# pgriewank/SAMSIM

Hardware: AMD Instinct MI355X
Metric: column-timesteps/sec (higher is better)
Workload: dtype f64

## Files before the change

samsim_amd/csrc/samsim_probe.h:

```cpp
#ifndef SAMSIM_PROBE_H
#define SAMSIM_PROBE_H

#ifndef SAMSIM_STAMPS
#define SAMSIM_STAMPS 0
#endif
#ifdef SAMSIM_ISA_MARKS
#define ISA_MARK(name) asm volatile("; ISA_MARK " name)
#else
#define ISA_MARK(name) ((void)0)
#endif
#if SAMSIM_STAMPS
__device__ unsigned long long g_stamps[48];
extern "C" int samsim_debug_stamps(unsigned long long *out, int reset) {
  if (out && hipMemcpyFromSymbol(out, HIP_SYMBOL(g_stamps), sizeof(unsigned long long) * 48) != hipSuccess) return -1;
  if (reset) { unsigned long long z[48] = {0}; if (hipMemcpyToSymbol(HIP_SYMBOL(g_stamps), z, sizeof(z)) != hipSuccess) return -1; }
  return 0;
}
#endif

namespace {

#if SAMSIM_STAMPS
enum { ST_PRO = 0, ST_DFUSED, ST_DUNFUSED, ST_SURF, ST_UP, ST_POST, ST_HEAD, ST_TAIL,
       CT_WAVESTEPS = 8, CT_FUSED, CT_UNFUSED, CT_UP_TRIPS, CT_NEWTON_WAVE, CT_NEWTON_LANE, CT_LANES, CT_DOWN_TRIPS, CT_DRAIN_WAVE,
       CT_DRAIN_LANE, CT_DIRTY, CT_L_COUPLING, ST_U_HEAD = 20, ST_U_GETT, ST_U_TAIL, ST_D_A, ST_D_B,
       CT_L_FLOODP = 25, CT_L_IRREG, CT_L_DIRTY, CT_L_UNFUSED, CT_L_FLUSH3, CT_L_REGRID, CT_L_FREEBOARD,
       CT_REFILL = 32, CT_ROWS, CT_ROWS_STILL, CT_ODD_LANES, CT_ODD_WAVES, CT_ODD_EVALS_WAVE, CT_LITE, ST_NSLOT = 48 };
struct Stamps {
  unsigned long long *acc;
  unsigned long long t0;
};
__device__ __forceinline__ bool st_leader() { return (int)__lane_id() == __ffsll((long long)__ballot(1)) - 1; }
__device__ __forceinline__ void st_mark(Stamps &st, int region) {
#if SAMSIM_STAMPS == 1
  const unsigned long long t = __builtin_amdgcn_s_memtime();
  if (st_leader()) st.acc[region] += t - st.t0;
  st.t0 = t;
#endif
}
__device__ __forceinline__ void st_count(Stamps &st, int counter, unsigned long long n = 1) {
#if SAMSIM_STAMPS == 2
  if (st_leader()) st.acc[counter] += n;
#endif
}
#define ST_MARK(r) st_mark(x.st, r)
#define ST_COUNT(cn, n) st_count(x.st, cn, n)
#else
#define ST_MARK(r) ((void)0)
#define ST_COUNT(cn, n) ((void)0)
#endif

}

#endif
```

samsim_amd/csrc/samsim_sweeps_fused.h:

```cpp
#ifndef SAMSIM_SWEEPS_FUSED_H
#define SAMSIM_SWEEPS_FUSED_H

namespace {


struct RayScan {
  double minp, stp, st;
  double bot, botterm, perm_bot, S_br_bot;
  double buoy_s, min_psi_s;
};
__device__ __forceinline__ void ray_scan_init(RayScan &r) {
  r.minp = 1.0e300; r.stp = 0.0; r.st = 0.0; r.bot = 0.0; r.botterm = 0.0; r.perm_bot = 0.0; r.S_br_bot = 0.0;
  r.buoy_s = 0.0; r.min_psi_s = 1.0e300;
}

struct Expelled { double psi_s, psi_l, psi_g, V_ex; };
__device__ __forceinline__ Expelled expulsion(double phi, double thick, double m, double rth) {
  Expelled e;
  const double V_s = m * phi * (1.0 / rho_s), V_l = m * (1.0 - phi) * (1.0 / rho_l);
  e.V_ex = dmax(V_l + V_s - thick, 0.0);
  e.psi_s = V_s * rth;
  e.psi_l = (V_l - e.V_ex) * rth;
  e.psi_g = (thick - V_l - V_s + e.V_ex) * rth;
  e.psi_l = dmax(e.psi_l, 0.0);
  e.psi_g = dmax(e.psi_g, 0.0);
  return e;
}

template <class K>
__device__ __forceinline__ void s1_layer(Col &c, const Ctx &x, int k, int Na, bool do_ray, double T, double phi, double S_bu,
                                         double m, double thick, double rth, RayScan &r, bool sparse_rows = false, const double *S_br_T = nullptr) {
  const samsim_config &g = x.p->cfg;
  const double S_br = S_br_T ? *S_br_T : S_br_clamped(x.salt, T, S_bu);
  const Expelled e = expulsion(phi, thick, m, rth);
  r.min_psi_s = dmin(r.min_psi_s, e.psi_s);
  r.buoy_s += e.psi_s * thick;
  if (k == 1) c.psi_l_top = e.psi_l;
  if (do_ray) {
    const double perm = x.p17 * pow_3p1(1000.0 * fabs(e.psi_l));
    if (k == Na) {
      r.S_br_bot = S_br;
      r.bot = thick * e.psi_s / psi_s_min;
      r.perm_bot = perm;
      r.botterm = r.bot / perm;
    } else {
      const double height = r.st + r.bot;
      r.minp = dmin(r.minp, perm);
      r.stp = r.stp + quot(thick, perm);
      r.st = r.st + thick;
      double ray;
      const double d_S_br = S_br - r.S_br_bot;
      if (CFG(harmonic_flag) == 2) {
        const double hp = (r.minp < x.p14) ? 0.0 : quot(r.st + r.bot, r.stp + r.botterm);
        ray = grav_f * rho_l * bbeta * d_S_br * height * hp;
      } else {
        ray = grav_f * rho_l * bbeta * d_S_br * height * dmin(r.minp, r.perm_bot);
      }
      ray = ray * (1.0 / (kappa_l * mu));
      ray = dmax(ray, 0.0);
      if (!sparse_rows) {
        LAYU(SAMSIM_A_RAY, k) = ray;
      } else if (k == 1 || x.ray_rows_all || wave_any(ray > ray_crit)) {
        LAYU(SAMSIM_A_RAY, k) = ray;
        x.rflag[(k - 1) >> 6] = x.rflag[(k - 1) >> 6] | (1ull << ((k - 1) & 63));
      }
    }
  }
}

template <class K>
__device__ __forceinline__ void flood_handover(Col &c, const Ctx &x, const RayScan &all, const RayScan &below_top, double thick_bottom) {
  const samsim_config &g = x.p->cfg;
  if (!(CFG(flood_flag) > 1 && c.Na > 1 && CL(m_snow) > all.buoy_s * (rho_l - rho_s))) return;
  SPEC(SP_FL_HP) = quot(all.st + all.bot, all.stp + all.botterm);
  SPEC(SP_FL_SALL) = all.st + thick_bottom;
  SPEC(SP_MINP) = below_top.minp; SPEC(SP_STP) = below_top.stp; SPEC(SP_ST) = below_top.st;
  SPEC(SP_BOT) = below_top.bot; SPEC(SP_BOTTERM) = below_top.botterm; SPEC(SP_SBR_BOT) = below_top.S_br_bot;
}

template <class K>
__device__ __forceinline__ void prologue_top_layer(Col &c, const Ctx &x) {
  const samsim_config &g = x.p->cfg;
  const int Na = c.Na;
  const bool do_ray = (CFG(grav_flag) >= 2 && Na > 1);
  RayScan r;
  r.minp = SPEC(SP_MINP); r.stp = SPEC(SP_STP); r.st = SPEC(SP_ST);
  r.bot = SPEC(SP_BOT); r.botterm = SPEC(SP_BOTTERM); r.perm_bot = SPEC(SP_PERM_BOT);
  r.S_br_bot = SPEC(SP_SBR_BOT); r.buoy_s = SPEC(SP_BUOY_S); r.min_psi_s = SPEC(SP_MIN_PSI_S);
  const RayScan r_below_top = r;
  const double H_abs = LAY(SAMSIM_A_H_ABS, 1), m = LAY(SAMSIM_A_M, 1), thick = LAY(SAMSIM_A_THICK, 1);
  double S_abs = LAY(SAMSIM_A_S_ABS, 1);
  if (S_abs < 0.0) { S_abs = 0.0; LAY(SAMSIM_A_S_ABS, 1) = S_abs; }
  double S_bu, H;
  per_mass(S_abs, H_abs, m, S_bu, H);
  if (K::general && CFG(prescribe_flag) == 2) LAY(SAMSIM_A_S_BU, 1) = S_abs / m;
  const double T_test = (Na > 1) ? LAY(SAMSIM_A_T, 2) : g.T_bottom;
  double T, phi = 0.0;
  const int rc = getT_chain(x.salt, H, S_bu, T_test, T, phi);
  LAY(SAMSIM_A_T, 1) = T;
  LAY(SAMSIM_A_PHI, 1) = phi;
  s1_layer<K>(c, x, 1, Na, do_ray, T, phi, S_bu, m, thick, recip(thick), r);
  if (do_ray && CFG(flood_flag) > 1 && CL(m_snow) > r.buoy_s * (rho_l - rho_s)) {
    THICK_RULE_INIT(tr);
    flood_handover<K>(c, x, r, r_below_top, THICK_AT(tr, Na));
  }
  c.neg_psi = r.min_psi_s < 0.0;
  c.buoy_s = r.buoy_s;
  if (rc) STOPC(rc, 1);
}

template <class K>
__device__ RARE void sweep_beer(Col &c, const Ctx &x, double beer0) {
  const samsim_config &g = x.p->cfg;
  const int Na = c.Na;
  if (!wave_any(beer0 != 0.0)) { c.frad = 0.0; return; }
  if ((c.flags & COLF_REGULAR) != 0) {
    const int n0 = __builtin_amdgcn_readfirstlane(Na);
    const bool same = !wave_any(Na != n0);
    const int kend = same ? n0 : wave_max(Na);
    const int b0 = g.n_top, b1 = g.n_top + g.n_middle;
    double temp2 = beer0, frad = 0.0;
#pragma unroll 1
    for (int st = 0; st < 4; ++st) {
      const int klo = st == 0 ? 1 : (st == 1 ? 2 : (st == 2 ? b0 + 1 : b1 + 1));
      const int khi_s = st == 0 ? 1 : (st == 1 ? b0 : (st == 2 ? b1 : kend));
      if (klo > kend) break;
      if (klo > khi_s) continue;
      const int khi = khi_s < kend ? khi_s : kend;
      const double thick = st == 0 ? LAYU(SAMSIM_A_THICK, 1) : (st == 2 ? LAYU(SAMSIM_A_THICK, g.n_top + 1) : g.thick_0);
      const double e = exp(-extinc * thick);
      if (same) {
        const int kmul = khi < kend ? khi : kend - 1;
        for (int k = klo; k <= kmul; ++k) temp2 = temp2 * e;
        if (khi == kend) frad = temp2 - temp2 * e;
      } else {
        for (int k = klo; k <= khi; ++k) {
          const double t = temp2 * e;
          if (k == Na) frad = temp2 - t;
          temp2 = t;
        }
      }
    }
    c.frad = frad;
  } else {
    double temp2 = beer0, e = 0.0, th_prev = -1.0;
    for (int k = 1; k <= Na; ++k) {
      const double thick = LAYU(SAMSIM_A_THICK, k);
      if (thick != th_prev) { e = exp(-extinc * thick); th_prev = thick; }
      if (k == Na) c.frad = temp2 - temp2 * e;
      temp2 = temp2 * e;
    }
  }
}

__device__ __forceinline__ double heat_conductance(double psi_s, double psi_l, double rth) {
  return (2.0 * (psi_s * k_s + psi_l * k_l)) * rth;
}
__device__ __forceinline__ double heat_flux_between(double dT, double g_a, double g_b) {
  return quot(dT * (g_a * g_b), g_a + g_b);
}

__device__ __forceinline__ double out_of_row(double v) {
#if defined(__HIP_DEVICE_COMPILE__)
  double r;
  asm volatile("v_mov_b64 %0, %1" : "=v"(r) : "v"(v));
  return r;
#else
  return v;
#endif
}

template <class K>
__device__ __forceinline__ void sweep_down_fused(Col &c, const Ctx &x, bool store_default, bool decide_psi, bool &surface_done,
                                                 bool couple, bool late_rad, double time, int tc, bool do_beer) {
  const samsim_config &g = x.p->cfg;
  const Salt &s = x.salt;
  const int Na = c.Na;
  const double dt = g.dt;
  double heat_loss = 0.0, cum = 0.0, sum_before = 0.0, sum_after = 0.0, minS = 1.0e300;
  double fb_a2 = 0.0, fb_g2 = 0.0;
  int stop_layer = 0;
  bool store_psi = true;
  double g_up = 0.0, flq_up = 0.0;
  double esum = 0.0;

  struct Ld { double T, S_abs, m, H_abs, ray; };
  struct Raw { double T, S_abs, m, S_bu, S_br, H_abs, ray, H; };
  auto load_ld = [&](int j) -> Ld {
    Ld r;
    r.T = LAYU_LD(SAMSIM_A_T, j);
    r.S_abs = LAYU_LD(SAMSIM_A_S_ABS, j);
    r.m = LAYU_LD(SAMSIM_A_M, j);
    r.H_abs = LAYU_LD(SAMSIM_A_H_ABS, j);
    r.ray = (j <= Na - 1 && ray_row_valid(c, x, j)) ? LAYU(SAMSIM_A_RAY, j) : 0.0;
    return r;
  };
  auto finish = [&](const Ld &l, int j) -> Raw {
    Raw r;
    r.T = l.T; r.S_abs = l.S_abs; r.m = l.m; r.H_abs = l.H_abs; r.ray = l.ray;
    per_mass(r.S_abs, r.H_abs, r.m, r.S_bu, r.H);
    r.S_br = S_br_clamped(s, r.T, r.S_bu);
    return r;
  };
  auto S_br_below = [&](const Ld &l) -> double {
    double S_bu, H;
    per_mass(l.S_abs, l.H_abs, l.m, S_bu, H);
    return S_br_clamped(s, l.T, S_bu);
  };
  struct Lay { double T, SA, mA, S_abs, H_abs, m, flup; bool ch; };

  double flm_j = 0.0;
  double T_up = 0.0, S_br_up = 0.0, S_abs_up = 0.0;
  const int N = c.N;
  Raw raw = finish(load_ld(1), 1);
  Ld ahead = load_ld(2), ahead2 = ahead;
  Lay prev = {0, 0, 1, 0, 0, 0, 0, true};
  double flup_pp = 0.0;
  auto layer = [&](const int j, const Ld &below, const double thick, const double rth, auto last_tag, auto first_tag) {
    constexpr bool LAST = decltype(last_tag)::value, FIRST = decltype(first_tag)::value;
    if (!LAST && !FIRST) { ISA_MARK("D_LAYER_A"); }
    double H_abs = raw.H_abs;
    const Expelled ex = expulsion(phi_from_T(s, raw.H, raw.S_bu, raw.S_br), thick, raw.m, rth);
    const double V_ex = ex.V_ex;
    double psi_g = ex.psi_g, m = raw.m, S_abs = raw.S_abs;
    const double T = raw.T, S_br = raw.S_br;
    double flm_next;
    if (j == 1 || psi_g < (double)0.001f) {
      flm_next = (j == 1) ? -V_ex * rho_l : -V_ex * rho_l + flm_j;
    } else {
      flm_next = -dmax((V_ex - psi_g * thick) * rho_l, 0.0);
      psi_g = dmax(quot(psi_g * thick - V_ex, thick), 0.0);
    }
    if (!FIRST) { fb_a2 += ex.psi_s * thick; fb_g2 += psi_g * thick; }
    if (store_psi || j == 1) {
      LAYU(SAMSIM_A_PSI_S, j) = ex.psi_s;
      LAYU(SAMSIM_A_PSI_L, j) = ex.psi_l;
      LAYU(SAMSIM_A_PSI_G, j) = psi_g;
    }
    const bool flooded_here = FIRST && (c.flags & COLF_FLOODED) != 0;
    const double th_l = flooded_here ? LAYU(SAMSIM_A_THICK, 1) : thick;
    const double gj = heat_conductance(ex.psi_s, ex.psi_l, flooded_here ? recip(th_l) : rth);
    const double flq = (j >= 2) ? heat_flux_between(T - prev.T, g_up, gj) : 0.0;
    if (j == 2) c.flq2 = flq;
    m = m + flm_next - flm_j;
    if (flm_next < 0.0) {
      H_abs = H_abs + flm_next * T * c_l;
      S_abs = S_abs + dmax(flm_next * S_br, -S_abs);
    }
    if (flm_j < 0.0) {
      H_abs = H_abs - flm_j * T_up * c_l;
      S_abs = S_abs - dmax(flm_j * S_br_up, -S_abs_up);
    }
    bool ch = LAST || (flm_next < 0.0) || (flm_j < 0.0);
#if SAMSIM_STAMPS == 2
    if (!LAST && !FIRST) {
      ST_COUNT(CT_ROWS, 1);
      if (__ballot(flm_next < 0.0 || flm_j < 0.0) == 0ull) ST_COUNT(CT_ROWS_STILL, 1);
    }
#endif
    const double SA = S_abs, mA = m;
    S_br_up = S_br;
    flm_j = flm_next;
    double Tl = T;
    if (FIRST && couple) {
      double phi1 = LAYU(SAMSIM_A_PHI, 1);
      const double S_bu1 = S_abs / m;
      LAYU(SAMSIM_A_S_BU, 1) = S_bu1;
      const int rcc = snow_coupling_core<K>(c, x, H_abs, m, S_bu1, Tl, phi1);
      LAYU(SAMSIM_A_T, 1) = Tl;
      LAYU(SAMSIM_A_PHI, 1) = phi1;
      if (rcc && !c.status) { c.status = rcc; x.err_step[c.col] = c.step + 1; x.err_layer[c.col] = 1; }
    }
    if (flooded_here) {
      S_abs = SPEC(SP_FLD_S1); H_abs = SPEC(SP_FLD_H1); m = SPEC(SP_FLD_M1);
      ch = true;
      c.flags &= ~COLF_FLOODED;
    }
    if (LAST) {
      if (psi_g > 0.0) {
        const double t2 = psi_g * thick * rho_l;
        m = m + t2;
        S_abs = S_abs + t2 * x.S_bu_bottom;
        H_abs = H_abs + t2 * c_l * g.T_bottom;
      }
      if (c.flags & COLF_FLOOD_DEEP) {
        S_abs = S_abs + SPEC(SP_FL_HP);
        H_abs = H_abs + SPEC(SP_FL_SALL);
        c.flags &= ~COLF_FLOOD_DEEP;
      }
      if (CFG(turb_flag) == 2) {
        const double turb = Turb_A * exp(Turb_B * (-ocean_density<K>(x) + func_density(T, quot(S_abs, m)))) * dt;
        S_abs = S_abs - turb * (S_abs / m - x.S_bu_bottom);
      }
    }
    if (!LAST && !FIRST) { ISA_MARK("D_LAYER_B"); }
    ST_MARK(ST_D_A);
    sum_before += S_abs;
    double flup = cum;
    if (!LAST) {
      const double ray = raw.ray;
      if (ray > ray_crit && S_br > S_br_below(below)) {
        const double psi_s = ex.psi_s;
        if (psi_s > 0.001 && (flooded_here ? quot(S_abs, m) : quot(SA, mA)) > 0.1) {
          ST_COUNT(CT_DRAIN_WAVE, 1);
          ST_COUNT(CT_DRAIN_LANE, (unsigned long long)__popcll(__ballot(1)));
          const double psi_l = ex.psi_l;
          double flux = x_grav * (ray - ray_crit) * dt * th_l;
          flux = dmin(flux, psi_l * rho_l * th_l);
          S_abs = S_abs - flux * S_br;
          if (S_abs < 0.0 && !stop_layer) stop_layer = j;
          CL(grav_temp) = CL(grav_temp) + flux * Tl;
          H_abs = H_abs - flux * c_l * Tl;
          heat_loss = heat_loss + flux * c_l * Tl;
          cum = cum + flux;
          flup = dmin(cum, psi_l * rho_l * th_l);
          ch = true;
        }
      }
    }
    sum_after += S_abs;
#if defined(__HIP_DEVICE_COMPILE__)
    asm volatile("" : "+v"(sum_before), "+v"(sum_after));
#endif
    if (!LAST && !FIRST) { ISA_MARK("D_LAYER_C"); }
    if (j > 1) {
      if (prev.flup > 0.0) {
        prev.H_abs = prev.H_abs + prev.flup * T * c_l;
        prev.S_abs = prev.S_abs + dmin(prev.flup * S_br_clamped(s, T, quot(SA, mA)), S_abs);
        prev.ch = true;
      }
      if (flup_pp > 0.0) {
        prev.H_abs = prev.H_abs - flup_pp * prev.T * c_l;
        prev.S_abs = prev.S_abs - dmin(flup_pp * S_br_clamped(s, prev.T, quot(prev.SA, prev.mA)), prev.S_abs);
        prev.ch = true;
      }
      if (j - 1 >= 2) {
        const double H_b = prev.H_abs;
        prev.H_abs = prev.H_abs + (flq - flq_up) * dt;
        prev.H_abs = prev.H_abs + c.frad * dt;
        esum += H_b - prev.H_abs;
      }
      if (wave_any(prev.ch)) {
        LAYU(SAMSIM_A_M, j - 1) = prev.m;
        LAYU(SAMSIM_A_S_ABS, j - 1) = prev.S_abs;
      }
      LAYU(SAMSIM_A_H_ABS, j - 1) = prev.H_abs;
      minS = dmin(minS, prev.S_abs);
      flup_pp = prev.flup;
    }
    g_up = gj; flq_up = flq;
    T_up = out_of_row(T); S_abs_up = out_of_row(SA);
    prev.T = FIRST ? out_of_row(Tl) : T_up; prev.SA = S_abs_up; prev.mA = mA; prev.S_abs = out_of_row(S_abs); prev.H_abs = out_of_row(H_abs);
    prev.m = m; prev.flup = flup; prev.ch = ch;
    if (!LAST && !FIRST) { ISA_MARK("D_LAYER_END"); }
    ST_MARK(ST_D_B);
  };
  const int jmax = wave_max(Na);
  auto request = [&](const int j) { ahead2 = load_ld(j + 2 <= N ? j + 2 : N); };
  auto advance = [&](const int j) { raw = finish(ahead, j + 1); ahead = ahead2; };
  const double thick1 = (c.flags & COLF_FLOODED) ? SPEC(SP_FLD_TH1_BEFORE) : LAYU(SAMSIM_A_THICK, 1);
  if (1 < Na) { request(1); layer(1, ahead, thick1, recip(thick1), std::false_type{}, std::true_type{}); advance(1); }
  if (2 < Na) { request(2); layer(2, ahead, g.thick_0, recip(g.thick_0), std::false_type{}, std::false_type{}); advance(2); }
  if (late_rad) {
    const double beer0 = radiation_header<K>(c, x, time, tc);
    c.frad = 0.0;
    if (do_beer) sweep_beer<K>(c, x, beer0);
  }
  if (decide_psi && Na >= 3) {
    surface_flux<K>(c, x);
    surface_done = true;
    const double thick_min = g.thick_min;
    const double Tf = func_T_freeze(quot(LAYU(SAMSIM_A_S_ABS, 1), LAYU(SAMSIM_A_M, 1)), CFG(salt_flag), x.tf_c3);
    bool snow_wet = false;
    if (CL(thick_snow) > 0.0) {
      const double H_new = CL(H_abs_snow) + (CL(fl_Q1) - CL(fl_Q_snow)) * dt;
      snow_wet = !(CL(thick_snow) >= thick_min) || !(H_new / CL(m_snow) <= -latent_heat);
    }
    store_psi = store_default || LAYU(SAMSIM_A_PSI_S, 1) < psi_s_top_min || CL(T_top) >= Tf || snow_wet || CL(melt_thick_snow) > 0.0;
  } else {
    store_psi = store_default || decide_psi;
  }
  c.psi_full = store_psi;
  {
    const int b0 = g.n_top, b1 = g.n_top + g.n_middle;
    Ld ahead3 = ahead;
    auto single = [&](const int j, const double th_s, const double rth_s) {
      ahead2 = load_ld(j + 2 <= N ? j + 2 : N);
      layer(j, ahead, th_s, rth_s, std::false_type{}, std::false_type{});
      raw = finish(ahead, j + 1);
      ahead = ahead2;
    };
    int j = 3;
    for (int stretch = 0; stretch < 3; ++stretch) {
      const int hi_s = stretch == 0 ? b0 : (stretch == 1 ? b1 : N);
      const int hi = hi_s < jmax - 1 ? hi_s : jmax - 1;
      const double th_s = stretch == 1 ? LAYU(SAMSIM_A_THICK, g.n_top + 1) : g.thick_0, rth_s = recip(th_s);
      for (; j + 2 <= hi; j += 3) {
        ISA_MARK("D_ITER_BEGIN");
        ST_MARK(ST_DFUSED);
        if (j + 2 < Na) {
          ST_COUNT(CT_DOWN_TRIPS, 3);
          ahead2 = load_ld(j + 2 <= N ? j + 2 : N);
          layer(j, ahead, th_s, rth_s, std::false_type{}, std::false_type{});
          raw = finish(ahead, j + 1);
          ahead3 = load_ld(j + 3 <= N ? j + 3 : N);
          layer(j + 1, ahead2, th_s, rth_s, std::false_type{}, std::false_type{});
          raw = finish(ahead2, j + 2);
          ahead = load_ld(j + 4 <= N ? j + 4 : N);
          layer(j + 2, ahead3, th_s, rth_s, std::false_type{}, std::false_type{});
          raw = finish(ahead3, j + 3);
        } else if (j < Na) {
          ISA_MARK("D_RARE_BEGIN");
          ST_COUNT(CT_DOWN_TRIPS, 1);
          single(j, th_s, rth_s);
          if (j + 1 < Na) { ST_COUNT(CT_DOWN_TRIPS, 1); single(j + 1, th_s, rth_s); }
        }
        ISA_MARK("D_ITER_END");
      }
      for (; j <= hi; ++j) {
        if (j < Na) single(j, th_s, rth_s);
      }
    }
  }
  const double thick_Na = (Na > g.n_top && Na <= g.n_top + g.n_middle) ? LAYU(SAMSIM_A_THICK, g.n_top + 1) : g.thick_0;
  layer(Na, ahead, thick_Na, recip(thick_Na), std::true_type{}, std::false_type{});
  if (prev.flup > 0.0) {
    prev.H_abs = prev.H_abs + prev.flup * g.T_bottom * c_l;
    prev.S_abs = prev.S_abs + dmin(prev.flup * S_br_clamped(s, g.T_bottom, x.S_bu_bottom), x.S_bu_bottom * 2000.0);
  }
  if (flup_pp > 0.0) {
    prev.H_abs = prev.H_abs - flup_pp * prev.T * c_l;
    prev.S_abs = prev.S_abs - dmin(flup_pp * S_br_clamped(s, prev.T, quot(prev.SA, prev.mA)), prev.S_abs);
  }
  CL(grav_drain) = CL(grav_drain) + prev.flup;
  if (CFG(grav_heat_flag) == 2) prev.H_abs = prev.H_abs + heat_loss - prev.flup * c_l * g.T_bottom;
  {
    const double H_b = prev.H_abs;
    prev.H_abs = prev.H_abs + (c.fl_q_bottom - flq_up) * dt;
    prev.H_abs = prev.H_abs + c.frad * dt;
    c.esum = esum + (H_b - prev.H_abs);
  }
  LAYU(SAMSIM_A_M, Na) = prev.m;
  LAYU(SAMSIM_A_S_ABS, Na) = prev.S_abs;
  LAYU(SAMSIM_A_H_ABS, Na) = prev.H_abs;
  minS = dmin(minS, prev.S_abs);
  if (store_psi) { SPEC(SP_FB_A2) = fb_a2; SPEC(SP_FB_G2) = fb_g2; }
  CL(grav_salt) = CL(grav_salt) + sum_before;
  CL(grav_salt) = CL(grav_salt) - sum_after;
  if (stop_layer) STOPC(21234, stop_layer);
  if (minS < 0.0) STOPC(1337, 0);
}

template <class K>
__device__ __forceinline__ void sweep_up_fused(Col &c, const Ctx &x, long long col, bool next_is_output, bool store_phi) {
  const samsim_config &g = x.p->cfg;
  const Salt &s = x.salt;
  const int Na = c.Na;
  const double dt = g.dt, thick_min = g.thick_min;
  const bool thin_snow = (CL(thick_snow) >= thick_min / 100.0 && CL(thick_snow) < thick_min);
  const bool do_ray = (CFG(grav_flag) >= 2 && Na > 1);
  const bool keep_ray = next_is_output && col >= x.out_col0 && col < x.out_col0 + x.out_ncols;
  const double H_abs_snow_before = CL(H_abs_snow);
  double esum = c.esum;
  double T_test = g.T_bottom;
  int rc = 0, rc_layer = 0;
  RayScan r;
  ray_scan_init(r);
  if (keep_ray) {
    const size_t oc = (size_t)(col - x.out_col0), on = (size_t)x.out_ncols;
    for (int k = 1; k <= c.N - 1; ++k) x.out_lay[((size_t)SAMSIM_A_RAY * c.N + (k - 1)) * on + oc] = LAYU(SAMSIM_A_RAY, k);
  }
  for (int w = 0; w <= (c.N - 1) >> 6; ++w) x.rflag[w] = 0ull;
  __builtin_amdgcn_wave_barrier();
  if (do_ray && Na <= c.N - 1 && x.ray_rows_all) LAYU(SAMSIM_A_RAY, Na) = 0.0;
  struct UL { double th, H, m, S; };
  const bool regular_wave = !wave_any((c.flags & COLF_REGULAR) == 0);
  UL cur, nxt, nn;
  bool alive = true, neg_salt = false;
  auto body = [&](const int k, const UL &row, const double th_k, const double rth_k, auto top_tag, auto lite_tag) {
    constexpr bool TOP = decltype(top_tag)::value;
    constexpr bool LITE = decltype(lite_tag)::value;
    const double H_k = row.H, m_k = row.m, S_k = row.S;
    double H_abs = H_k;
    const double m = m_k;
    if (TOP) {
      const double flq_below = (Na >= 2) ? c.flq2 : c.fl_q_bottom;
      const double H_b = H_abs;
      H_abs = H_abs + (flq_below - CL(fl_Q1)) * dt;
      H_abs = H_abs + c.frad * dt;
      if (thin_snow) {
        CL(H_abs_snow) = CL(H_abs_snow) - CL(fl_Q_snow) * dt;
        LAYU(SAMSIM_A_H_ABS, 1) = H_abs;
        snow_coupling<K>(c, x);
        if (c.status) { alive = false; return; }
        H_abs = LAYU(SAMSIM_A_H_ABS, 1);
      } else if (CL(thick_snow) >= thick_min) {
        CL(H_abs_snow) = CL(H_abs_snow) + (CL(fl_Q1) - CL(fl_Q_snow)) * dt;
      }
      esum += H_b - H_abs;
      LAYU(SAMSIM_A_H_ABS, 1) = H_abs;
    }
    double S_abs = S_k;
    double S_bu, H;
    per_mass(S_abs, H_abs, m, S_bu, H);
    double T, phi = 0.0, S_br_T = 0.0;
    if (!TOP) { ISA_MARK("U_GETT_BEGIN"); }
    ST_MARK(ST_U_HEAD);
#if SAMSIM_STAMPS == 2
    int evals = 1;
    int rr = TOP ? getT(s, H, S_bu, T_test, T, phi, &evals) : getT_chain<LITE>(s, H, S_bu, T_test, T, phi, &evals, LITE ? nullptr : &S_br_T);
    {
      const bool was_odd = (evals >> 30) & 1;
      const int redo = (evals >> 16) & 0x3fff;
      evals &= 0xffff;
      const unsigned long long om = __ballot(was_odd);
      if (om) { ST_COUNT(CT_ODD_LANES, (unsigned long long)__popcll(om)); ST_COUNT(CT_ODD_WAVES, 1); ST_COUNT(CT_ODD_EVALS_WAVE, (unsigned long long)wave_max(redo)); }
    }
    ST_COUNT(CT_UP_TRIPS, 1);
    ST_COUNT(CT_NEWTON_WAVE, (unsigned long long)wave_max(evals));
    { int tot = 0; unsigned long long mk = __ballot(1); while (mk) { const int ln = __ffsll((long long)mk) - 1; tot += __builtin_amdgcn_readlane(evals, ln); mk &= mk - 1; }
      ST_COUNT(CT_NEWTON_LANE, (unsigned long long)tot); }
#else
    int rr = TOP ? getT(s, H, S_bu, T_test, T, phi) : getT_chain<LITE>(s, H, S_bu, T_test, T, phi, nullptr, LITE ? nullptr : &S_br_T);
#endif
    if (!TOP) { ISA_MARK("U_GETT_END"); }
    ST_MARK(ST_U_GETT);
    if (rr && !rc) { rc = rr; rc_layer = k; }
    T_test = T;
    LAYU(SAMSIM_A_T, k) = T;
    if (store_phi || TOP || k >= Na - 1) LAYU(SAMSIM_A_PHI, k) = phi;
    if (!TOP && !LITE) {
      neg_salt = neg_salt || (S_abs < 0.0);
      s1_layer<K>(c, x, k, Na, do_ray, T, phi, S_bu, m, th_k, rth_k, r, true, &S_br_T);
    }
    ST_MARK(ST_U_TAIL);
  };
  const int kmax = wave_max(Na);
  auto load3 = [&](int j) -> UL { UL u; u.th = 0.0; u.H = LAYU_LD(SAMSIM_A_H_ABS, j); u.m = LAYU_LD(SAMSIM_A_M, j); u.S = LAYU_LD(SAMSIM_A_S_ABS, j); return u; };
  auto load4 = [&](int j) -> UL { UL u = load3(j); u.th = LAYU(SAMSIM_A_THICK, j); return u; };
  auto layers = [&](auto lite_tag) {
  if (regular_wave) {
    const int kc = kmax >= 2 ? kmax - 1 : 1;
    UL a = load3(kmax), b = load3(kc), d = b;
    auto one = [&](const int k, const UL &row, UL &req, const double th_s, const double rth_s) {
      req = load3(k >= 3 ? k - 2 : 1);
      if (k <= Na) body(k, row, th_s, rth_s, std::false_type{}, lite_tag);
    };
    const int b0 = g.n_top, b1 = g.n_top + g.n_middle;
    int k = kmax;
    for (int stretch = 0; stretch < 3; ++stretch) {
      const int klo = stretch == 0 ? b1 + 1 : (stretch == 1 ? b0 + 1 : 2);
      const double th_s = stretch == 1 ? LAYU(SAMSIM_A_THICK, g.n_top + 1) : g.thick_0, rth_s = recip(th_s);
      for (; k - 2 >= klo; k -= 3) {
        ISA_MARK("U_ITER_BEGIN");
        ST_MARK(ST_UP);
        one(k, a, d, th_s, rth_s);
        ISA_MARK("U_LAYER_2");
        one(k - 1, b, a, th_s, rth_s);
        ISA_MARK("U_LAYER_3");
        one(k - 2, d, b, th_s, rth_s);
        ISA_MARK("U_ITER_END");
      }
      for (; k >= klo; --k) {
        ISA_MARK("U_REST_BEGIN");
        ST_MARK(ST_UP);
        one(k, a, d, th_s, rth_s);
        a = b; b = d;
        ISA_MARK("U_REST_END");
      }
    }
    cur = a;
  } else {
    cur = load4(Na); nxt = load4(Na >= 2 ? Na - 1 : 1); nn = nxt;
    for (int k = kmax; k >= 2; --k) {
      if (k > Na) continue;
      nn = load4(k >= 3 ? k - 2 : 1);
      body(k, cur, cur.th, recip(cur.th), std::false_type{}, lite_tag);
      cur = nxt; nxt = nn;
    }
  }
  };
  const bool lite = K::fixed && CFG(flush_flag) == 5 && wave_any((c.flags & COLF_FLUSHED) != 0);
  if (lite) { ST_COUNT(CT_LITE, 1); layers(std::true_type{}); } else layers(std::false_type{});
  __builtin_amdgcn_wave_barrier();
  if (neg_salt || lite) c.flags |= COLF_DIRTY;
  body(1, cur, LAYU(SAMSIM_A_THICK, 1), 0.0, std::true_type{}, std::false_type{});
  if (!alive) return;
  if (!lite) {
  SPEC(SP_MINP) = r.minp; SPEC(SP_STP) = r.stp; SPEC(SP_ST) = r.st;
  SPEC(SP_BOT) = r.bot; SPEC(SP_BOTTERM) = r.botterm; SPEC(SP_PERM_BOT) = r.perm_bot;
  SPEC(SP_SBR_BOT) = r.S_br_bot; SPEC(SP_BUOY_S) = r.buoy_s; SPEC(SP_MIN_PSI_S) = r.min_psi_s;
  }
  double bal = esum + (H_abs_snow_before - CL(H_abs_snow));
  bal = bal + (double)Na * (c.frad * dt);
  if (thin_snow || CL(thick_snow) >= thick_min) bal = bal + c.fl_q_bottom * dt - CL(fl_Q_snow) * dt;
  else bal = bal + c.fl_q_bottom * dt - CL(fl_Q1) * dt;
  if (fabs(bal / dt) > 0.00001) STOPC(431, 0);
  if (rc) STOPC(rc, rc_layer);
}

}

#endif
```

samsim_amd/csrc/samsim_thermo.h:

```cpp
#ifndef SAMSIM_THERMO_H
#define SAMSIM_THERMO_H

namespace {

#include "samsim_div.h"
#if defined(__HIP_DEVICE_COMPILE__)
__device__ __forceinline__ double dmax(double a, double b) {
  double r;
  if (__builtin_constant_p(b) && b == 0.0) asm("v_max_f64 %0, %1, 0" : "=v"(r) : "v"(a));
  else asm("v_max_f64 %0, %1, %2" : "=v"(r) : "v"(a), "v"(b));
  return r;
}
__device__ __forceinline__ double dmin(double a, double b) {
  double r;
  asm("v_min_f64 %0, %1, %2" : "=v"(r) : "v"(a), "v"(b));
  return r;
}
#else
__device__ __forceinline__ double dmax(double a, double b) { return a > b ? a : b; }
__device__ __forceinline__ double dmin(double a, double b) { return a < b ? a : b; }
#endif
#if defined(__HIP_DEVICE_COMPILE__)
__device__ __forceinline__ double fma_c(double a, double b, double c_const) {
  double r;
  asm("v_fma_f64 %0, %1, %2, %3" : "=v"(r) : "v"(a), "v"(b), "s"(c_const));
  return r;
}
__device__ __forceinline__ double max_c(double a, double c_const) {
  double r;
  asm("v_max_f64 %0, %1, %2" : "=v"(r) : "v"(a), "s"(c_const));
  return r;
}
#else
__device__ __forceinline__ double fma_c(double a, double b, double c_const) { return __builtin_fma(a, b, c_const); }
__device__ __forceinline__ double max_c(double a, double c_const) { return a > c_const ? a : c_const; }
#endif
__device__ __forceinline__ void per_mass(double S_abs, double H_abs, double m, double &S_bu, double &H) {
  const double rm = recip(m);
  S_bu = S_abs * rm;
  H = H_abs * rm;
}

__device__ __forceinline__ double S_br_poly(const Salt &s, double T) {
  return T * (s.c2 + T * (s.c3 + T * s.c4));
}
__device__ __forceinline__ double S_br_clamped(const Salt &s, double T, double S_bu) {
  double v = S_br_poly(s, T);
  return dmax(v, S_bu);
}
__device__ __forceinline__ double ddT_S_br(const Salt &s, double T) {
  const double T_crit = -20.0;
  double d = s.d2 + 2.0 * s.d3 * T + 3.0 * s.d4 * (T * T);
  if (T < T_crit) d = s.d2 + 2.0 * s.d3 * T_crit + 3.0 * s.d4 * (T_crit * T_crit);
  return d;
}

__device__ __forceinline__ void newton_terms(const Salt &s, double H, double S_bu, double T_0, double sb, double sb_floor,
                                             double &f, double &ddT_f) {
  if (sb > 0.0001) {
    const double inv = recip(sb);
    f = -latent_heat - H + latent_heat * S_bu * inv + c_s * T_0 + c_s_beta * T_0 * T_0 / 2.0;
    ddT_f = c_s + c_s_beta * T_0 - latent_heat * S_bu * ddT_S_br(s, T_0) * (inv * inv);
    return;
  }
  f = -latent_heat - H + latent_heat * S_bu / dmax(sb, sb_floor) + c_s * T_0 + c_s_beta * T_0 * T_0 / 2.0;
  ddT_f = c_s + c_s_beta * T_0 - latent_heat * S_bu * ddT_S_br(s, T_0) / dmax(sb * sb, 0.0000000001);
}

struct NewtonConsts { double c3, cs, d3x2; };
__device__ __forceinline__ NewtonConsts newton_consts(const Salt &s) {
  NewtonConsts n = {s.c3, c_s, 2.0 * s.d3};
#if defined(__HIP_DEVICE_COMPILE__)
  asm volatile("" : "+v"(n.c3), "+v"(n.cs), "+v"(n.d3x2));
#endif
  return n;
}
__device__ __forceinline__ void newton_eval(const Salt &s, const NewtonConsts &n, double A0, double LS, double T_0, double &T_new, bool &more, bool &ok) {
  const double sbf = T_0 * fma_c(T_0, __builtin_fma(T_0, s.c4, n.c3), s.c2);
  const double sb2 = sbf * sbf;
  const double A = __builtin_fma(T_0, __builtin_fma(T_0, 0.5 * c_s_beta, n.cs), A0);
  const double B = __builtin_fma(c_s_beta, T_0, n.cs);
  const double num = __builtin_fma(A, sb2, LS * sbf);
  const double Tc = max_c(T_0, -20.0);
  const double dd = fma_c(Tc, __builtin_fma(Tc, 3.0 * s.d4, n.d3x2), s.d2);
  const double den = __builtin_fma(B, sb2, -(LS * dd));
  T_new = T_0 - quot(num, den);
  more = fabs(num) > sb2;
  ok = sbf > 0.0001;
}

__device__ __forceinline__ bool newton_step(const Salt &s, double H, double S_bu, double T_0, double sb_floor, double &T_new) {
  {
    bool more, ok;
    double Tn;
    newton_eval(s, newton_consts(s), -latent_heat - H, latent_heat * S_bu, T_0, Tn, more, ok);
    if (ok) { T_new = Tn; return more; }
  }
  const double sb = S_br_poly(s, T_0);
  double f, ddT_f;
  newton_terms(s, H, S_bu, T_0, sb, sb_floor, f, ddT_f);
  T_new = T_0 - quot(f, ddT_f);
  return fabs(f) > 1.0;
}

__device__ __forceinline__ double T_liquid(double H) {
  return H * (1.0 / c_l);
}

__device__ __forceinline__ double T_freeze_of(const Salt &s, double S_bu) {
  double T_fr = -1.0;
  while (fabs(S_br_poly(s, T_fr) / S_bu - 1.0) > (double)0.0001f) {
    const double t0 = T_fr;
    T_fr = t0 - (S_br_poly(s, t0) - S_bu) / ddT_S_br(s, t0);
  }
  return T_fr;
}

__device__ __forceinline__ int getT(const Salt &s, double H, double S_bu, double T_in, double &T_out, double &phi_out, int *evals = nullptr) {
  double T = T_liquid(H), phi = phi_out;
  int rc = 0;
  if (S_br_clamped(s, T, S_bu) > S_bu && S_bu > 0.001) {
    double T_fr = 0.0, T_0;
    bool have_T_fr = false;
    T_0 = T_in;
    bool more = newton_step(s, H, S_bu, T_0, 0.000000001, T);
    int i = 0;
    while (more) {
      T_0 = T;
      if (T_0 > 0.0 || T_0 < -200.0) {
        if (!have_T_fr) {
          T_fr = T_freeze_of(s, S_bu);
          have_T_fr = true;
        }
        T_0 = T_fr;
      }
      more = newton_step(s, H, S_bu, T_0, 0.0000000001, T);
#if SAMSIM_STAMPS == 2
      if (evals) *evals += 1;
#endif
      if (++i == 260) { rc = 99; break; }
    }
    phi = 1.0 - quot(S_bu, S_br_clamped(s, T, S_bu));
  } else if (S_bu < 0.001) {
    if (H > 0.0) { phi = 0.0; T = H / c_l; }
    else if (H <= -latent_heat) { phi = 1.0; T = (H + latent_heat) / c_s; }
    else if (H <= 0.0 && -latent_heat < H) { T = 0.0; phi = -H / latent_heat; }
  } else {
    phi = 0.0;
  }
  T_out = T;
  phi_out = phi;
  return rc;
}

template <bool WARM = false>
__device__ __forceinline__ int getT_chain(const Salt &s, double H, double S_bu, double T_in, double &T_out, double &phi_out, int *evals = nullptr,
                                          double *S_br_out = nullptr) {
  const double Tl = T_liquid(H);
  const bool above = S_br_clamped(s, Tl, S_bu) > S_bu, salty = S_bu > 0.001;
  const double A0 = -latent_heat - H, LS = latent_heat * S_bu;
  const NewtonConsts nc = newton_consts(s);
  double T;
  bool more0, ok;
  newton_eval(s, nc, A0, LS, T_in, T, more0, ok);
  unsigned long long odd_m = __builtin_amdgcn_ballot_w64(!above) | __builtin_amdgcn_ballot_w64(!salty) | __builtin_amdgcn_ballot_w64(!ok);
  unsigned long long more_m = __builtin_amdgcn_ballot_w64(more0) & ~odd_m;
  int i = 0;
  double T_fr = 0.0;
  bool have_T_fr = false;
  ISA_MARK("NEWTON_LOOP");
  for (;;) {
    if (more_m == 0ull) break;
    const bool more = __builtin_amdgcn_inverse_ballot_w64(more_m);
    if (WARM) {
      const unsigned long long out_m = more_m & (__builtin_amdgcn_ballot_w64(T > 0.0) | __builtin_amdgcn_ballot_w64(T < -200.0));
      if (out_m != 0ull) {
        if (__builtin_amdgcn_inverse_ballot_w64(out_m)) {
          if (!have_T_fr) { T_fr = T_freeze_of(s, S_bu); have_T_fr = true; }
          T = T_fr;
        }
      }
    }
    double Tn;
    bool m2, ok2;
    newton_eval(s, nc, A0, LS, T, Tn, m2, ok2);
    unsigned long long left_m = __builtin_amdgcn_ballot_w64(!ok2);
    if (!WARM) left_m |= __builtin_amdgcn_ballot_w64(T > 0.0) | __builtin_amdgcn_ballot_w64(T < -200.0);
    const unsigned long long m2_m = __builtin_amdgcn_ballot_w64(m2);
#if SAMSIM_STAMPS == 2
    if (evals && more) *evals += 1;
#endif
    T = more ? Tn : T;
    odd_m |= left_m & more_m;
    more_m &= m2_m & ~left_m;
    if (++i == 260) { odd_m |= more_m; break; }
  }
  const bool odd = __builtin_amdgcn_inverse_ballot_w64(odd_m);
  ISA_MARK("NEWTON_LOOP_END");
  double phi = S_br_out ? 0.0 : 1.0 - quot(S_bu, S_br_clamped(s, T, S_bu));
  int rc = 0;
  if (odd) {
    phi = phi_out;
#if SAMSIM_STAMPS == 2
    int ev0 = evals ? *evals : 0;
#endif
    rc = getT(s, H, S_bu, T_in, T, phi, evals);
#if SAMSIM_STAMPS == 2
    if (evals) *evals += ((*evals - ev0) << 16) | (1 << 30);
#endif
  }
  if (S_br_out) {
    const double S_br_T = S_br_clamped(s, T, S_bu);
    if (!odd) phi = 1.0 - quot(S_bu, S_br_T);
    *S_br_out = S_br_T;
  }
  T_out = T;
  phi_out = phi;
  return rc;
}

__device__ __forceinline__ double phi_from_T(const Salt &s, double H, double S_bu, double S_br_T) {
  if (S_bu > 0.001) return 1.0 - quot(S_bu, S_br_T);
  if (S_bu < 0.001) {
    if (H > 0.0) return 0.0;
    if (H <= -latent_heat) return 1.0;
    return -H / latent_heat;
  }
  return 0.0;
}

}
#define SP_QUOT(a, b) quot(a, b)
#include "samsim_pow.h"
namespace {
__device__ __forceinline__ double pow_3p1(double x) { return sp_pow_3p1(x); }

__device__ __forceinline__ double pow_1p5(double x) { return sp_pow_1p5(x); }
__device__ __forceinline__ double pow_4(double x) { return sp_pow_4(x); }

__device__ double func_density(double T, double S) {
  double density_0 = 999.842594 + 6.8 / 100.0 * T;
  return density_0 + 0.825 * S + (-5.7 / 1000.0) * pow_1p5(dmax(S, 0.0));
}

__device__ double func_T_freeze(double S_bu, int salt_flag, double tf_c3) {
  if (salt_flag == 2) {
    return -0.0592 * S_bu - (double)9.37f * (S_bu * S_bu) - tf_c3 * (S_bu * S_bu * S_bu);
  } else {
    const float a = 1.710523f * 1e-3f, b = 2.154996f * 1e-4f;
    return -0.0575 * S_bu + (double)a * pow_1p5(S_bu) - (double)b * (S_bu * S_bu);
  }
}

__device__ double func_albedo(double thick_snow, double T_snow, double psi_l, double thick_min, int albedo_flag) {
  const double ice_dry = (double)0.75f, ice_wet = (double)0.6f, snow_dry = (double)0.85f, snow_wet = (double)0.75f,
               water = (double)0.2f;
  double albedo;
  if (thick_snow > thick_min) {
    albedo = (T_snow < (double)(-0.01f)) ? snow_dry : snow_wet;
    albedo = ice_dry + (albedo - ice_dry) * dmin(1.0, quot(thick_snow, 0.3));
  } else {
    if (psi_l > 0.9) albedo = water;
    else if (psi_l > 0.6) albedo = ice_wet + (water - ice_wet) * ((psi_l - 0.6) / 0.3);
    else if (psi_l > 0.2) albedo = ice_wet;
    else albedo = ice_dry;
  }
  if (albedo_flag == 1) {
    if (thick_snow > thick_min) albedo = (T_snow < (double)(-0.01f)) ? snow_dry : snow_wet;
    else albedo = (psi_l < (double)0.8f) ? ice_dry : water;
  }
  return albedo;
}

__device__ double func_k_snow(double m_snow, double thick_snow) {
  const double c0 = 0.138, c1 = -1.01 / 1000.0, c2 = 3.233 / 1000000.0;
  double r = quot(m_snow, thick_snow);
  double k_snow = c0 + quot(c1 * m_snow, thick_snow) + c2 * (r * r);
  return k_snow + (double)0.15f;
}

__device__ __forceinline__ double time_input(int k) { return ((double)(float)k - 1.0) * 3600.0 * 3.0; }

template <class K>
__device__ __forceinline__ double ocean_density(const Ctx &x) {
  if ((K::fixed ? K::tank_flag : x.p->cfg.tank_flag) == 2 || (K::sites && x.ocean_sbu)) return func_density(x.p->cfg.T_bottom, x.S_bu_bottom);
  return x.rho_bottom;
}

}

#endif
```

Baseline: 764.4 million.

## Skip bounded Rayleigh rows, shortcut brine check, hoist Newton constants

In the ray scan, sparse harmonic rows now use a division-free wave-wide bound test (P < Q) and return early, before the quotient and store, when no lane can exceed the critical Rayleigh number. In getT_chain, the brine-salinity check is skipped wave-wide when every lane has a liquidus temperature below -3 and bulk salinity below 40, on the assumption that the check cannot fail in that range. Newton constants are computed once per stretch and passed in rather than recomputed on every call. Together these cut per-layer arithmetic in the upward sweep, at the cost of relying on the bound and the shortcut being exact for all inputs, and of a little extra branching.

```diff
diff --git a/samsim_amd/csrc/samsim_probe.h b/samsim_amd/csrc/samsim_probe.h
--- a/samsim_amd/csrc/samsim_probe.h
+++ b/samsim_amd/csrc/samsim_probe.h
@@ -25,7 +25,8 @@
        CT_WAVESTEPS = 8, CT_FUSED, CT_UNFUSED, CT_UP_TRIPS, CT_NEWTON_WAVE, CT_NEWTON_LANE, CT_LANES, CT_DOWN_TRIPS, CT_DRAIN_WAVE,
        CT_DRAIN_LANE, CT_DIRTY, CT_L_COUPLING, ST_U_HEAD = 20, ST_U_GETT, ST_U_TAIL, ST_D_A, ST_D_B,
        CT_L_FLOODP = 25, CT_L_IRREG, CT_L_DIRTY, CT_L_UNFUSED, CT_L_FLUSH3, CT_L_REGRID, CT_L_FREEBOARD,
-       CT_REFILL = 32, CT_ROWS, CT_ROWS_STILL, CT_ODD_LANES, CT_ODD_WAVES, CT_ODD_EVALS_WAVE, CT_LITE, ST_NSLOT = 48 };
+       CT_REFILL = 32, CT_ROWS, CT_ROWS_STILL, CT_ODD_LANES, CT_ODD_WAVES, CT_ODD_EVALS_WAVE, CT_LITE,
+       CT_RAY_ROWS = 39, CT_RAY_ROWS_BOUND, CT_ABOVE_ROWS, CT_ABOVE_FAST, ST_NSLOT = 48 };
 struct Stamps {
   unsigned long long *acc;
   unsigned long long t0;
diff --git a/samsim_amd/csrc/samsim_sweeps_fused.h b/samsim_amd/csrc/samsim_sweeps_fused.h
--- a/samsim_amd/csrc/samsim_sweeps_fused.h
+++ b/samsim_amd/csrc/samsim_sweeps_fused.h
@@ -50,8 +50,19 @@
       r.st = r.st + thick;
       double ray;
       const double d_S_br = S_br - r.S_br_bot;
-      if (CFG(harmonic_flag) == 2) {
-        const double hp = (r.minp < x.p14) ? 0.0 : quot(r.st + r.bot, r.stp + r.botterm);
+      const bool harmonic = CFG(harmonic_flag) == 2;
+      const double h_sum = harmonic ? r.st + r.bot : 0.0, h_den = harmonic ? r.stp + r.botterm : 0.0;
+      if (sparse_rows && harmonic && k != 1 && !x.ray_rows_all) {
+        constexpr double q_ray = ray_crit * (1.0 - 0x1p-20) * (kappa_l * mu);
+        const double P = grav_f * rho_l * bbeta * d_S_br * height * h_sum, Q = q_ray * h_den;
+        ST_COUNT(CT_RAY_ROWS, 1);
+        if ((__builtin_amdgcn_ballot_w64(!(P < Q)) & __builtin_amdgcn_ballot_w64(!(r.minp < x.p14))) == 0ull) {
+          ST_COUNT(CT_RAY_ROWS_BOUND, 1);
+          return;
+        }
+      }
+      if (harmonic) {
+        const double hp = (r.minp < x.p14) ? 0.0 : quot(h_sum, h_den);
         ray = grav_f * rho_l * bbeta * d_S_br * height * hp;
       } else {
         ray = grav_f * rho_l * bbeta * d_S_br * height * dmin(r.minp, r.perm_bot);
@@ -477,6 +488,7 @@
   const bool regular_wave = !wave_any((c.flags & COLF_REGULAR) == 0);
   UL cur, nxt, nn;
   bool alive = true, neg_salt = false;
+  NewtonConsts nc_s = newton_consts(s);
   auto body = [&](const int k, const UL &row, const double th_k, const double rth_k, auto top_tag, auto lite_tag) {
     constexpr bool TOP = decltype(top_tag)::value;
     constexpr bool LITE = decltype(lite_tag)::value;
@@ -508,8 +520,10 @@
     ST_MARK(ST_U_HEAD);
 #if SAMSIM_STAMPS == 2
     int evals = 1;
-    int rr = TOP ? getT(s, H, S_bu, T_test, T, phi, &evals) : getT_chain<LITE>(s, H, S_bu, T_test, T, phi, &evals, LITE ? nullptr : &S_br_T);
+    int rr = TOP ? getT(s, H, S_bu, T_test, T, phi, &evals) : getT_chain<LITE>(s, H, S_bu, T_test, T, phi, &evals, LITE ? nullptr : &S_br_T, &nc_s);
     {
+      if (!TOP) { ST_COUNT(CT_ABOVE_ROWS, 1); if (__ballot(evals < 0)) ST_COUNT(CT_ABOVE_FAST, 1); }
+      evals &= 0x7fffffff;
       const bool was_odd = (evals >> 30) & 1;
       const int redo = (evals >> 16) & 0x3fff;
       evals &= 0xffff;
@@ -521,7 +535,7 @@
     { int tot = 0; unsigned long long mk = __ballot(1); while (mk) { const int ln = __ffsll((long long)mk) - 1; tot += __builtin_amdgcn_readlane(evals, ln); mk &= mk - 1; }
       ST_COUNT(CT_NEWTON_LANE, (unsigned long long)tot); }
 #else
-    int rr = TOP ? getT(s, H, S_bu, T_test, T, phi) : getT_chain<LITE>(s, H, S_bu, T_test, T, phi, nullptr, LITE ? nullptr : &S_br_T);
+    int rr = TOP ? getT(s, H, S_bu, T_test, T, phi) : getT_chain<LITE>(s, H, S_bu, T_test, T, phi, nullptr, LITE ? nullptr : &S_br_T, &nc_s);
 #endif
     if (!TOP) { ISA_MARK("U_GETT_END"); }
     ST_MARK(ST_U_GETT);
@@ -551,6 +565,7 @@
     for (int stretch = 0; stretch < 3; ++stretch) {
       const int klo = stretch == 0 ? b1 + 1 : (stretch == 1 ? b0 + 1 : 2);
       const double th_s = stretch == 1 ? LAYU(SAMSIM_A_THICK, g.n_top + 1) : g.thick_0, rth_s = recip(th_s);
+      nc_s = newton_consts(s);
       for (; k - 2 >= klo; k -= 3) {
         ISA_MARK("U_ITER_BEGIN");
         ST_MARK(ST_UP);
diff --git a/samsim_amd/csrc/samsim_thermo.h b/samsim_amd/csrc/samsim_thermo.h
--- a/samsim_amd/csrc/samsim_thermo.h
+++ b/samsim_amd/csrc/samsim_thermo.h
@@ -155,15 +155,21 @@
 
 template <bool WARM = false>
 __device__ __forceinline__ int getT_chain(const Salt &s, double H, double S_bu, double T_in, double &T_out, double &phi_out, int *evals = nullptr,
-                                          double *S_br_out = nullptr) {
+                                          double *S_br_out = nullptr, const NewtonConsts *nc_in = nullptr) {
   const double Tl = T_liquid(H);
-  const bool above = S_br_clamped(s, Tl, S_bu) > S_bu, salty = S_bu > 0.001;
+  const bool salty = S_bu > 0.001;
   const double A0 = -latent_heat - H, LS = latent_heat * S_bu;
-  const NewtonConsts nc = newton_consts(s);
+  const NewtonConsts nc = nc_in ? *nc_in : newton_consts(s);
+  const bool short_cut = (__builtin_amdgcn_ballot_w64(!(Tl < -3.0)) | __builtin_amdgcn_ballot_w64(!(S_bu < 40.0))) == 0ull;
+  unsigned long long brine_m = 0ull;
+  if (!short_cut) brine_m = __builtin_amdgcn_ballot_w64(!(S_br_clamped(s, Tl, S_bu) > S_bu));
+#if SAMSIM_STAMPS == 2
+  if (short_cut && evals) *evals = (int)((unsigned)*evals | 0x80000000u);
+#endif
   double T;
   bool more0, ok;
   newton_eval(s, nc, A0, LS, T_in, T, more0, ok);
-  unsigned long long odd_m = __builtin_amdgcn_ballot_w64(!above) | __builtin_amdgcn_ballot_w64(!salty) | __builtin_amdgcn_ballot_w64(!ok);
+  unsigned long long odd_m = brine_m | __builtin_amdgcn_ballot_w64(!salty) | __builtin_amdgcn_ballot_w64(!ok);
   unsigned long long more_m = __builtin_amdgcn_ballot_w64(more0) & ~odd_m;
   int i = 0;
   double T_fr = 0.0;
```

After: 776.3 million, median of 6. +1.6%, better.
